# StefanDenn3r/Unsupervised_Anomaly_Detection_Brain_MRI

Hardware: AMD Instinct MI355X
Metric: MRI slices/sec VAE train step (128x128, bs=64) (higher is better)
Workload: dtype bf16x3; 1 GPU; BASELINE.json configs[1]: VAE 128x128x1 slices, batch 64 per GPU, fwd + bwd + TF-Adam (lr 1e-4, beta1 0.5), dropout 0.2, inter_res 8, zDim 128; global_batch=64, per_gpu_batch=64, parallelism=single

## Files before the change

unsupervised_anomaly_detection_brain_mri_amd/csrc/uad_misc.hip:

```cpp
#include "uad_kernels.h"
#include <stdint.h>

namespace {

__device__ __forceinline__ float wave_sum(float v) {
#pragma unroll
    for (int o = 32; o > 0; o >>= 1) v += __shfl_xor(v, o);
    return v;
}

typedef float v4f_nt __attribute__((ext_vector_type(4)));
template <int JL, int SL>
__device__ __forceinline__ void reduce4_block(v4f_nt (*red)[JL], int vb, const float* __restrict__ partial, int S, int L, float scale, float* __restrict__ out) {
    const int jl = threadIdx.x % JL, sl = threadIdx.x / JL;
    const int j4 = vb * JL + jl, L4 = L >> 2;
    v4f_nt a0 = {0.f, 0.f, 0.f, 0.f}, a1 = a0, a2 = a0, a3 = a0;
    if (j4 < L4) {
        const v4f_nt* p = reinterpret_cast<const v4f_nt*>(partial) + j4;
        int s = sl;
        for (; s + 3 * SL < S; s += 4 * SL) {
            const v4f_nt v0 = __builtin_nontemporal_load(p + (size_t)s * L4), v1 = __builtin_nontemporal_load(p + (size_t)(s + SL) * L4);
            const v4f_nt v2 = __builtin_nontemporal_load(p + (size_t)(s + 2 * SL) * L4), v3 = __builtin_nontemporal_load(p + (size_t)(s + 3 * SL) * L4);
            a0 += v0; a1 += v1; a2 += v2; a3 += v3;
        }
// ... 261 lines not shown
    else if constexpr (SLAB == RF_VEC16) reduce4_block<16, 32>(reinterpret_cast<v4f_nt (*)[16]>(lds), vb, a.partial, a.S, a.L, 1.0f, a.dW);
    else if constexpr (SLAB == RF_SCALAR4) reduce1_block<128, 4>(reinterpret_cast<float (*)[128]>(lds), vb, a.partial, a.S, a.L, 1.0f, a.dW, 1);
    else if constexpr (SLAB == RF_SCALAR16) reduce1_block<32, 16>(reinterpret_cast<float (*)[32]>(lds), vb, a.partial, a.S, a.L, 1.0f, a.dW, 1);
}

__global__ void __launch_bounds__(256) colsum_kernel(const float* __restrict__ g, int rows, int C, int rows_per_chunk,
                                                     float* __restrict__ out) {
    __shared__ float red[8][33];
    const int cl = threadIdx.x & 31, rl = threadIdx.x >> 5;
    const int c = blockIdx.x * 32 + cl;
    const int r0 = blockIdx.y * rows_per_chunk;
    const int r1 = min(r0 + rows_per_chunk, rows);
    float s = 0.f;
    if (c < C)
        for (int r = r0 + rl; r < r1; r += 8) s += g[(size_t)r * C + c];
    red[rl][cl] = s;
    __syncthreads();
    if (rl == 0 && c < C) {
        float a = 0.f;
        for (int k = 0; k < 8; ++k) a += red[k][cl];
        out[(size_t)blockIdx.y * C + c] = a;
    }
}

__global__ void __launch_bounds__(256) conv_first_fwd_kernel(UadConvDesc d, const float* __restrict__ x,
                                                             const float* __restrict__ W,
                                                             const float* __restrict__ bias, float* __restrict__ out) {
    extern __shared__ __attribute__((aligned(16))) float sm[];
    const int CS = d.CS, CB = d.CB, KS = d.KS, S = d.S, P = d.P;
    const int tpp = CS / 8;
    const int ppb = 256 / tpp;
    const int nwtaps = KS * KS * CB;
    float* ws = sm;
    const int xw = S * ppb + KS;
    float* xs = sm + nwtaps * CS;
    const int blocks_per_row = (d.WS + ppb - 1) / ppb;
    const int bx = blockIdx.x % blocks_per_row;
    const int row = blockIdx.x / blocks_per_row;
    const int n = row / d.HS, oy = row % d.HS;
    const int ox0 = bx * ppb;
    for (int i = threadIdx.x; i < nwtaps * CS; i += 256) ws[i] = W[i];
    const int ix0 = S * ox0 - P, iy0 = S * oy - P;
    for (int i = threadIdx.x; i < KS * xw * CB; i += 256) {
        const int cb = i % CB;
        const int t = i / CB;
        const int xx = t % xw, ky = t / xw;
        const int iy = iy0 + ky, ix = ix0 + xx;
        float v = 0.f;
        if ((unsigned)iy < (unsigned)d.HB && (unsigned)ix < (unsigned)d.WB)
            v = x[((size_t)(n * d.HB + iy) * d.WB + ix) * CB + cb];
        xs[i] = v;
    }
    __syncthreads();
    const int p = threadIdx.x / tpp, q = threadIdx.x % tpp;
    const int ox = ox0 + p;
    if (ox >= d.WS) return;
    float acc[8];
#pragma unroll
    for (int e = 0; e < 8; ++e) acc[e] = bias ? bias[q * 8 + e] : 0.f;
    for (int ky = 0; ky < KS; ++ky)
        for (int kx = 0; kx < KS; ++kx)
            for (int cb = 0; cb < CB; ++cb) {
                const float xv = xs[(ky * xw + S * p + kx) * CB + cb];
                const float4 w0 = *reinterpret_cast<const float4*>(ws + ((ky * KS + kx) * CB + cb) * CS + q * 8);
                const float4 w1 = *reinterpret_cast<const float4*>(ws + ((ky * KS + kx) * CB + cb) * CS + q * 8 + 4);
                acc[0] = fmaf(xv, w0.x, acc[0]); acc[1] = fmaf(xv, w0.y, acc[1]);
                acc[2] = fmaf(xv, w0.z, acc[2]); acc[3] = fmaf(xv, w0.w, acc[3]);
                acc[4] = fmaf(xv, w1.x, acc[4]); acc[5] = fmaf(xv, w1.y, acc[5]);
                acc[6] = fmaf(xv, w1.z, acc[6]); acc[7] = fmaf(xv, w1.w, acc[7]);
            }
    float* o = out + ((size_t)(n * d.HS + oy) * d.WS + ox) * CS + q * 8;
    *reinterpret_cast<float4*>(o) = make_float4(acc[0], acc[1], acc[2], acc[3]);
    *reinterpret_cast<float4*>(o + 4) = make_float4(acc[4], acc[5], acc[6], acc[7]);
}

template <int KS, int CB>
__global__ void __launch_bounds__(256) conv_first_wgrad_kernel(UadConvDesc d, const float* __restrict__ x,
                                                               const float* __restrict__ g, int rows_per_block,
                                                               float* __restrict__ partial) {
    extern __shared__ __attribute__((aligned(16))) float sm[];
    constexpr int NTAP = KS * KS * CB;
    const int CS = d.CS, S = d.S, P = d.P;
    const int G = 256 / CS;
    const int co = threadIdx.x % CS, grp = threadIdx.x / CS;
    const int xw = d.WB + KS + S;
    float* xs = sm;
    float acc[NTAP];
#pragma unroll
    for (int t = 0; t < NTAP; ++t) acc[t] = 0.f;
    const int total_rows = d.N * d.HS;
    const int row0 = blockIdx.x * rows_per_block;
    const int row1 = min(row0 + rows_per_block, total_rows);
    constexpr int RB = 4, OXB = 8;
    for (int rb = row0; rb < row1; rb += RB) {
        __syncthreads();
        for (int i = threadIdx.x; i < RB * KS * xw * CB; i += 256) {
            const int cb = i % CB;
            int t = i / CB;
            const int xx = t % xw; t /= xw;
            const int ky = t % KS, r = t / KS;
            const int row = rb + r;
            float v = 0.f;
            if (row < row1) {
                const int n = row / d.HS, oy = row % d.HS;
                const int iy = S * oy - P + ky, ix = xx - P;
                if ((unsigned)iy < (unsigned)d.HB && (unsigned)ix < (unsigned)d.WB)
                    v = x[((size_t)(n * d.HB + iy) * d.WB + ix) * CB + cb];
            }
            xs[i] = v;
        }
        __syncthreads();
        for (int ob = 0; ob < d.WS; ob += OXB * G) {
            float gv[RB][OXB];
#pragma unroll
            for (int r = 0; r < RB; ++r)
#pragma unroll
                for (int i = 0; i < OXB; ++i) {
                    const int ox = ob + grp + i * G;
                    const bool ok = (rb + r < row1) && ox < d.WS;
                    gv[r][i] = ok ? g[((size_t)(rb + r) * d.WS + ox) * CS + co] : 0.f;
                }
#pragma unroll
            for (int r = 0; r < RB; ++r)
#pragma unroll
                for (int i = 0; i < OXB; ++i) {
                    const int ox = min(ob + grp + i * G, d.WS - 1);
                    const float* xr = xs + (size_t)r * KS * xw * CB;
#pragma unroll
                    for (int ky = 0; ky < KS; ++ky)
#pragma unroll
                        for (int kx = 0; kx < KS; ++kx)
#pragma unroll
                            for (int cb = 0; cb < CB; ++cb)
                                acc[(ky * KS + kx) * CB + cb] =
                                    fmaf(xr[(ky * xw + S * ox + kx) * CB + cb], gv[r][i], acc[(ky * KS + kx) * CB + cb]);
                }
        }
    }
    __syncthreads();
    float* red = sm;
#pragma unroll
    for (int t = 0; t < NTAP; ++t) red[(grp * NTAP + t) * CS + co] = acc[t];
    __syncthreads();
    for (int i = threadIdx.x; i < NTAP * CS; i += 256) {
        float a = 0.f;
        for (int k = 0; k < G; ++k) a += red[k * NTAP * CS + i];
        partial[(size_t)blockIdx.x * NTAP * CS + i] = a;
    }
}

typedef float v2f __attribute__((ext_vector_type(2)));

template <int WS>
__global__ void __launch_bounds__(256) conv_first_fwd32_kernel(UadConvDesc d, const float* __restrict__ x, const float* __restrict__ W,
                                                               const float* __restrict__ bias, float* __restrict__ out) {
    constexpr int OR = 256 / WS, IR = 2 * OR + 3, XW = 2 * WS + 4;
    __shared__ __attribute__((aligned(16))) float ws[25 * 32];
    __shared__ __attribute__((aligned(16))) float xs[IR * XW];
    const int tid = threadIdx.x;
    const int q = tid & 3, pg = (tid >> 2) % (WS / 4), rl = tid / WS;
    const int bpi = d.HS / OR;
    const int n = blockIdx.x / bpi, oy0 = (blockIdx.x % bpi) * OR;
    for (int i = tid; i < 25 * 32; i += 256) ws[i] = W[i];
    for (int i = tid; i < IR * XW; i += 256) {
        const int r = i / XW, xx = i % XW;
        const int iy = 2 * oy0 - 1 + r, ix = xx - 1;
        xs[i] = ((unsigned)iy < (unsigned)d.HB && (unsigned)ix < (unsigned)d.WB) ? x[((size_t)n * d.HB + iy) * d.WB + ix] : 0.f;
    }
    __syncthreads();
    v2f acc[4][4];
#pragma unroll
    for (int e = 0; e < 4; ++e) {
        const v2f b = bias ? v2f{bias[q * 8 + 2 * e], bias[q * 8 + 2 * e + 1]} : v2f{0.f, 0.f};
#pragma unroll
        for (int j = 0; j < 4; ++j) acc[j][e] = b;
    }
    const float* xr0 = xs + (2 * rl) * XW + 8 * pg;
#pragma unroll
    for (int ky = 0; ky < 5; ++ky) {
        float xv[12];
#pragma unroll
        for (int k = 0; k < 3; ++k) *reinterpret_cast<float4*>(xv + 4 * k) = *reinterpret_cast<const float4*>(xr0 + ky * XW + 4 * k);
#pragma unroll
        for (int kx = 0; kx < 5; ++kx) {
            const float4 w0 = *reinterpret_cast<const float4*>(ws + (ky * 5 + kx) * 32 + q * 8);
            const float4 w1 = *reinterpret_cast<const float4*>(ws + (ky * 5 + kx) * 32 + q * 8 + 4);
            const v2f w[4] = {{w0.x, w0.y}, {w0.z, w0.w}, {w1.x, w1.y}, {w1.z, w1.w}};
#pragma unroll
            for (int j = 0; j < 4; ++j) {
                const v2f xx = {xv[2 * j + kx], xv[2 * j + kx]};
#pragma unroll
                for (int e = 0; e < 4; ++e) acc[j][e] = __builtin_elementwise_fma(xx, w[e], acc[j][e]);
            }
        }
    }
    const size_t oe = (((size_t)n * d.HS + oy0 + rl) * WS + 4 * pg) * 32 + q * 8;
    float* o = out + oe;
#pragma unroll
    for (int j = 0; j < 4; ++j) {
        *reinterpret_cast<float4*>(o + j * 32) = make_float4(acc[j][0].x, acc[j][0].y, acc[j][1].x, acc[j][1].y);
        *reinterpret_cast<float4*>(o + j * 32 + 4) = make_float4(acc[j][2].x, acc[j][2].y, acc[j][3].x, acc[j][3].y);
    }
}

template <int WS>
__global__ void __launch_bounds__(256) conv_first_wgrad32_kernel(UadConvDesc d, const float* __restrict__ x, const float* __restrict__ g,
                                                                 int RPB, float* __restrict__ partial) {
    constexpr int XW = 2 * WS + 4, NP = WS / 32, MAXR = 16;
    __shared__ __attribute__((aligned(16))) float xs[(2 * MAXR + 3) * XW];
    __shared__ __attribute__((aligned(16))) float red[4][25 * 32];
    const int tid = threadIdx.x, cq = tid & 7, pl = tid >> 3;
    const int row0 = blockIdx.x * RPB;
    const int n = row0 / d.HS, oy0 = row0 % d.HS;
    for (int i = tid; i < (2 * RPB + 3) * XW; i += 256) {
        const int r = i / XW, xx = i % XW;
        const int iy = 2 * oy0 - 1 + r, ix = xx - 1;
        xs[i] = ((unsigned)iy < (unsigned)d.HB && (unsigned)ix < (unsigned)d.WB) ? x[((size_t)n * d.HB + iy) * d.WB + ix] : 0.f;
    }
    v2f acc[25][2];
#pragma unroll
    for (int t = 0; t < 25; ++t) { acc[t][0] = v2f{0.f, 0.f}; acc[t][1] = v2f{0.f, 0.f}; }
    const float* gb = g + ((size_t)row0 * WS + pl) * 32 + cq * 4;
    float4 cur[2][NP], nxt[2][NP];
#pragma unroll
    for (int r = 0; r < 2; ++r)
#pragma unroll
        for (int k = 0; k < NP; ++k) cur[r][k] = *reinterpret_cast<const float4*>(gb + ((size_t)r * WS + k * 32) * 32);
    __syncthreads();
    for (int rp = 0; rp < RPB; rp += 2) {
        if (rp + 2 < RPB) {
#pragma unroll
            for (int r = 0; r < 2; ++r)
#pragma unroll
                for (int k = 0; k < NP; ++k) nxt[r][k] = *reinterpret_cast<const float4*>(gb + ((size_t)(rp + 2 + r) * WS + k * 32) * 32);
        }
#pragma unroll
        for (int r = 0; r < 2; ++r)
#pragma unroll
            for (int k = 0; k < NP; ++k) {
                const float* xr = xs + 2 * (rp + r) * XW + 2 * (k * 32 + pl);
                const v2f g0 = {cur[r][k].x, cur[r][k].y}, g1 = {cur[r][k].z, cur[r][k].w};
#pragma unroll
                for (int ky = 0; ky < 5; ++ky)
#pragma unroll
                    for (int kx = 0; kx < 5; ++kx) {
                        const float xv = xr[ky * XW + kx];
                        const v2f xx = {xv, xv};
                        acc[ky * 5 + kx][0] = __builtin_elementwise_fma(xx, g0, acc[ky * 5 + kx][0]);
                        acc[ky * 5 + kx][1] = __builtin_elementwise_fma(xx, g1, acc[ky * 5 + kx][1]);
                    }
            }
#pragma unroll
        for (int r = 0; r < 2; ++r)
#pragma unroll
            for (int k = 0; k < NP; ++k) cur[r][k] = nxt[r][k];
    }
#pragma unroll
    for (int t = 0; t < 25; ++t)
#pragma unroll
        for (int h = 0; h < 2; ++h) {
            float a = acc[t][h].x, b = acc[t][h].y;
            a += __shfl_xor(a, 8); b += __shfl_xor(b, 8);
            a += __shfl_xor(a, 16); b += __shfl_xor(b, 16);
            a += __shfl_xor(a, 32); b += __shfl_xor(b, 32);
            acc[t][h] = v2f{a, b};
        }
    const int wave = tid >> 6;
    if ((tid & 63) < 8) {
#pragma unroll
        for (int t = 0; t < 25; ++t)
            *reinterpret_cast<float4*>(&red[wave][t * 32 + cq * 4]) = make_float4(acc[t][0].x, acc[t][0].y, acc[t][1].x, acc[t][1].y);
    }
    __syncthreads();
    for (int i = tid; i < 25 * 32; i += 256) partial[(size_t)blockIdx.x * 800 + i] = (red[0][i] + red[1][i]) + (red[2][i] + red[3][i]);
}

template <bool BWD>
__global__ void __launch_bounds__(256) final_kernel(const UadFinalArgs a, int pix_per_block) {
    __shared__ float red[4][200];
    const int lpp = a.C / 4;
    const int ppp = 256 / lpp;
    const int cl = threadIdx.x % lpp, slot = threadIdx.x / lpp;
    const int n = blockIdx.y;
    const int hw = a.H * a.W;
    const int p0 = blockIdx.x * pix_per_block;
    const int p1 = min(p0 + pix_per_block, hw);
    float4 sc = *reinterpret_cast<const float4*>(a.scale + cl * 4);
    sc.x *= a.mult; sc.y *= a.mult; sc.z *= a.mult; sc.w *= a.mult;
    const float4 sh = *reinterpret_cast<const float4*>(a.shift + cl * 4);
    const float4 wf = *reinterpret_cast<const float4*>(a.wf + cl * 4);
    const float bf = a.bf[0];
    float rec = 0.f, dbf = 0.f;
    float dw[4] = {0, 0, 0, 0}, s1[4] = {0, 0, 0, 0}, s2[4] = {0, 0, 0, 0};
    constexpr int UNR = 4;
    auto one_pixel = [&](const size_t pix, const float4 c, const float xv) {
        float bn[4] = {fmaf(c.x, sc.x, sh.x), fmaf(c.y, sc.y, sh.y), fmaf(c.z, sc.z, sh.z), fmaf(c.w, sc.w, sh.w)};
        float av[4];
#pragma unroll
        for (int e = 0; e < 4; ++e) av[e] = bn[e] > 0.f ? bn[e] : bn[e] * a.alpha;
        float dot = av[0] * wf.x;
        dot = fmaf(av[1], wf.y, dot);
        dot = fmaf(av[2], wf.z, dot);
        dot = fmaf(av[3], wf.w, dot);
        for (int o = 1; o < lpp; o <<= 1) dot += __shfl_xor(dot, o);
        const float xh = dot + bf;
        const float diff = xh - xv;
        if (cl == 0) {
            a.x_hat[pix] = xh;
            if (a.l1_map) a.l1_map[pix] = fabsf(diff);
            rec += fabsf(diff);
        }
        if (BWD) {
            const float s = a.dxhat_in ? a.dxhat_in[pix] : (diff > 0.f ? 1.f : (diff < 0.f ? -1.f : 0.f)) * a.inv_batch;
            const float wv[4] = {wf.x, wf.y, wf.z, wf.w};
            const float cv[4] = {c.x, c.y, c.z, c.w};
            const float scv[4] = {sc.x, sc.y, sc.z, sc.w};
            float dc[4];
#pragma unroll
            for (int e = 0; e < 4; ++e) {
                const float da = s * wv[e];
                const float dbn = bn[e] > 0.f ? da : da * a.alpha;
                dc[e] = dbn * scv[e];
                dw[e] = fmaf(s, av[e], dw[e]);
                s1[e] += dbn;
                s2[e] = fmaf(dbn, cv[e], s2[e]);
            }
            *reinterpret_cast<float4*>(a.d_c + pix * a.C + cl * 4) = make_float4(dc[0], dc[1], dc[2], dc[3]);
            if (cl == 0) dbf += s;
        }
    };
    for (int p = p0 + slot; p < p1; p += ppp * UNR) {
        float4 cv[UNR];
        float xv[UNR];
#pragma unroll
        for (int u = 0; u < UNR; ++u) {
            const int pp = min(p + u * ppp, p1 - 1);
            const size_t pix = (size_t)n * hw + pp;
            cv[u] = *reinterpret_cast<const float4*>(a.c_last + pix * a.C + cl * 4);
            xv[u] = a.x[pix];
        }
#pragma unroll
        for (int u = 0; u < UNR; ++u)
            if (p + u * ppp < p1) one_pixel((size_t)n * hw + p + u * ppp, cv[u], xv[u]);
    }
    const int lane = threadIdx.x & 63, wave = threadIdx.x >> 6;
    for (int o = lpp; o < 64; o <<= 1) {
        rec += __shfl_xor(rec, o);
        if (BWD) {
            dbf += __shfl_xor(dbf, o);
#pragma unroll
            for (int e = 0; e < 4; ++e) {
                dw[e] += __shfl_xor(dw[e], o);
                s1[e] += __shfl_xor(s1[e], o);
                s2[e] += __shfl_xor(s2[e], o);
            }
        }
    }
    if (lane < lpp) {
        if (BWD) {
#pragma unroll
            for (int e = 0; e < 4; ++e) {
                red[wave][0 * a.C + lane * 4 + e] = dw[e];
                red[wave][1 * a.C + lane * 4 + e] = s1[e];
                red[wave][2 * a.C + lane * 4 + e] = s2[e];
            }
        }
        if (lane == 0) {
            red[wave][3 * a.C] = dbf;
            red[wave][3 * a.C + 1] = rec;
        }
    }
    __syncthreads();
    const int blk = blockIdx.y * gridDim.x + blockIdx.x;
    const int nred = 3 * a.C + 2;
    if ((int)threadIdx.x < nred) {
        const float v = red[0][threadIdx.x] + red[1][threadIdx.x] + red[2][threadIdx.x] + red[3][threadIdx.x];
        if ((int)threadIdx.x == 3 * a.C + 1) a.rec_partial[blk] = v;
        else if (BWD) a.red_partial[(size_t)blk * (3 * a.C + 1) + threadIdx.x] = v;
    }
}

__global__ void __launch_bounds__(64) reparam_fwd_kernel(int zdim, int n_vae, const float* __restrict__ mu_raw,
                                                         const float* __restrict__ ls_raw,
                                                         const float* __restrict__ mask_mu,
                                                         const float* __restrict__ mask_ls,
                                                         const float* __restrict__ mask_mu_ce,
                                                         const float* __restrict__ eps, float* __restrict__ mu,
                                                         float* __restrict__ ls, float* __restrict__ sigma,
                                                         float* __restrict__ z, float* __restrict__ kl) {
    const int n = blockIdx.x;
    const bool ctx = n >= n_vae;
    float acc = 0.f;
    for (int k = threadIdx.x; k < zdim; k += 64) {
        const size_t i = (size_t)n * zdim + k;
        float m = mu_raw[i];
        if (ctx) {
            if (mask_mu_ce) m *= mask_mu_ce[(size_t)(n - n_vae) * zdim + k];
            mu[i] = m; ls[i] = 0.f; sigma[i] = 1.f; z[i] = m;
            continue;
        }
        float l = ls_raw[i];
        if (mask_mu) m *= mask_mu[i];
        if (mask_ls) l *= mask_ls[i];
        const float s = expf(l);
        const float e = eps ? eps[i] : 0.f;
        mu[i] = m; ls[i] = l; sigma[i] = s;
        z[i] = fmaf(e, s, m);
        acc += m * m + s * s - 2.f * l - 1.f;
    }
    acc = wave_sum(acc);
    if (threadIdx.x == 0) kl[n] = 0.5f * acc;
}

__global__ void reparam_bwd_kernel(size_t total, int zdim, int n_vae, const float* __restrict__ dz,
                                   const float* __restrict__ mu, const float* __restrict__ sigma,
                                   const float* __restrict__ eps, const float* __restrict__ mask_mu,
                                   const float* __restrict__ mask_ls, const float* __restrict__ mask_mu_ce,
                                   float inv_batch, float* __restrict__ dmu_raw, float* __restrict__ dls_raw) {
    const size_t i = (size_t)blockIdx.x * blockDim.x + threadIdx.x;
    if (i >= total) return;
    const size_t n = i / zdim;
    const float g = dz[i];
    if (n >= (size_t)n_vae) {
        dmu_raw[i] = mask_mu_ce ? g * mask_mu_ce[i - (size_t)n_vae * zdim] : g;
        dls_raw[i] = 0.f;
// ... 303 lines not shown
namespace {
struct RngJobs { UadRngJob j[8]; };
__global__ void __launch_bounds__(256) rng_fill_kernel(RngJobs jobs, int n, unsigned k0, unsigned k1, unsigned step_lo, unsigned step_hi,
                                                       long long sample0) {
    const UadRngJob jb = jobs.j[blockIdx.y];
    const int quads = (jb.per_sample + 3) / 4;
    const long long total = (long long)n * quads;
    for (long long q = (long long)blockIdx.x * blockDim.x + threadIdx.x; q < total; q += (long long)gridDim.x * blockDim.x) {
        const int s = (int)(q / quads), e4 = (int)(q % quads);
        const unsigned long long gs = (unsigned long long)(sample0 + s);
        unsigned r[4];
        uad_rng_quad((unsigned)e4, gs, step_lo, step_hi, jb.stream, k0, k1, r);
        float v[4];
        if (jb.kind == 0) {
#pragma unroll
            for (int h = 0; h < 2; ++h) uad_box_muller(r[2 * h], r[2 * h + 1], v[2 * h], v[2 * h + 1]);
        } else {
            const float keep = 1.0f / (1.0f - jb.rate);
#pragma unroll
            for (int h = 0; h < 4; ++h) v[h] = ((float)(r[h] >> 8) * 5.9604644775390625e-8f >= jb.rate) ? keep : 0.0f;
        }
        float* o = jb.out + (size_t)s * jb.per_sample + (size_t)e4 * 4;
#pragma unroll
        for (int h = 0; h < 4; ++h) if (e4 * 4 + h < jb.per_sample) o[h] = v[h];
    }
}
}

void uad_launch_rng_fill(const UadRngJob* jobs, int njobs, int n, unsigned long long seed, unsigned long long step, long long sample0,
                         hipStream_t st) {
    RngJobs js;
    int maxq = 1;
    for (int i = 0; i < njobs; ++i) { js.j[i] = jobs[i]; const int q = (jobs[i].per_sample + 3) / 4; if (q > maxq) maxq = q; }
    long long blocks = ((long long)n * maxq + 255) / 256;
    if (blocks > 2048) blocks = 2048;
    hipLaunchKernelGGL(rng_fill_kernel, dim3((unsigned)blocks, njobs), dim3(256), 0, st, js, n, (unsigned)seed, (unsigned)(seed >> 32),
                       (unsigned)step, (unsigned)(step >> 32), sample0);
}

namespace {
__global__ void __launch_bounds__(64) clock_probe_kernel(unsigned long long* out, unsigned long long ticks) {
    const unsigned long long r0 = wall_clock64();
    const unsigned long long c0 = (unsigned long long)clock64();
    unsigned long long r = r0;
    while (r - r0 < ticks) { __builtin_amdgcn_s_sleep(64); r = wall_clock64(); }
    const unsigned long long c1 = (unsigned long long)clock64();
    if (threadIdx.x == 0) { out[0] = c1 - c0; out[1] = r - r0; }
}
}
void uad_launch_clock_probe(unsigned long long* out, unsigned long long ticks, hipStream_t st) {
    hipLaunchKernelGGL(clock_probe_kernel, dim3(1), dim3(64), 0, st, out, ticks);
}

void uad_launch_gather_slices(const float* src, const int* idx, int n, long long slice_elems, float* out, hipStream_t st) {
    const long long f4 = slice_elems / 4;
    int bx = (int)((f4 + 255) / 256); if (bx > 64) bx = 64; if (bx < 1) bx = 1;
    hipLaunchKernelGGL(gather_slices_kernel, dim3(bx, n), dim3(256), 0, st, src, idx, f4, out);
}
void uad_launch_gather_mask(const unsigned char* labels, const int* idx, int n, long long slice_px, const unsigned char* lut,
                            float* out, hipStream_t st) {
    int bx = (int)((slice_px + 255) / 256); if (bx > 64) bx = 64; if (bx < 1) bx = 1;
    hipLaunchKernelGGL(gather_mask_kernel, dim3(bx, n), dim3(256), 0, st, labels, idx, slice_px, lut, out);
}
static int reduce_form(const float* partial, int S, int L, const float* out) {
    static const bool r4 = getenv("UAD_NO_REDUCE4") == nullptr;
    if (r4 && S > 8 && L % 4 == 0 && L >= 1024 && ((uintptr_t)partial & 15) == 0 && ((uintptr_t)out & 15) == 0) {
        const int L4 = L / 4;
        return (L4 + 63) / 64 >= 256 ? RF_VEC64 : (L4 + 31) / 32 >= 256 ? RF_VEC32 : RF_VEC16;
    }
    return ((L + 63) / 64 >= 256 || S <= 8) ? RF_SCALAR4 : RF_SCALAR16;
}
void uad_launch_reduce_partials(const float* partial, int S, int L, float scale, float* out, hipStream_t st) {
    const int blocks = (L + 63) / 64, L4 = L / 4;
    constexpr int nt = 1;
    switch (reduce_form(partial, S, L, out)) {
    case RF_VEC64: hipLaunchKernelGGL((reduce_partials4_kernel<64, 8>), dim3((L4 + 63) / 64), dim3(512), 0, st, partial, S, L, scale, out); break;
    case RF_VEC32: hipLaunchKernelGGL((reduce_partials4_kernel<32, 16>), dim3((L4 + 31) / 32), dim3(512), 0, st, partial, S, L, scale, out); break;
    case RF_VEC16: hipLaunchKernelGGL((reduce_partials4_kernel<16, 32>), dim3((L4 + 15) / 16), dim3(512), 0, st, partial, S, L, scale, out); break;
    case RF_SCALAR4: hipLaunchKernelGGL((reduce_partials_kernel<4>), dim3(blocks), dim3(256), 0, st, partial, S, L, scale, out, nt); break;
    default: hipLaunchKernelGGL((reduce_partials_kernel<16>), dim3(blocks), dim3(1024), 0, st, partial, S, L, scale, out, nt); break;
    }
}

bool uad_grad_finish_takes(int C, int fin_C) { return C <= 512 && 3 * fin_C + 1 <= kFinishFinCols; }
size_t uad_grad_finish_scratch_floats() { return (size_t)kFinishBnFloats + 16 * kFinishFinCols; }
void uad_launch_grad_finish(const UadGradFinish& in, hipStream_t st) {
    UadGradFinish a = in;
    if (!a.fin_partial) a.fin_C = 0;
    if (!a.colpart) a.C = 0;
    if (!uad_grad_finish_takes(a.C, a.fin_C)) { fprintf(stderr, "uad: grad_finish does not take C = %d, fin_C = %d (uad_grad_finish_takes)\n", a.C, a.fin_C); abort(); }
    a.nfin = a.fin_partial ? (a.fin_T <= 8 ? 4 : 16) : 0;
    a.NB = a.T >= 2048 ? 32 : a.T >= 512 ? 16 : a.T >= 128 ? 8 : 1;
    a.nbn = a.colpart ? ((a.C + 31) / 32) * a.NB : 0;
    const int form = (a.partial && a.S > 0) ? reduce_form(a.partial, a.S, a.L, a.dW) : RF_NONE;
    const int L4 = a.L / 4;
    const int nslab = form == RF_VEC64 ? (L4 + 63) / 64 : form == RF_VEC32 ? (L4 + 31) / 32 : form == RF_VEC16 ? (L4 + 15) / 16
                      : form == RF_SCALAR4 ? (a.L + 127) / 128 : form == RF_SCALAR16 ? (a.L + 31) / 32 : 0;
    const dim3 grid(a.nfin + a.nbn + nslab);
    if (!grid.x) return;
    switch (form) {
    case RF_VEC64: hipLaunchKernelGGL(grad_finish_kernel<RF_VEC64>, grid, dim3(512), 0, st, a); break;
    case RF_VEC32: hipLaunchKernelGGL(grad_finish_kernel<RF_VEC32>, grid, dim3(512), 0, st, a); break;
    case RF_VEC16: hipLaunchKernelGGL(grad_finish_kernel<RF_VEC16>, grid, dim3(512), 0, st, a); break;
    case RF_SCALAR4: hipLaunchKernelGGL(grad_finish_kernel<RF_SCALAR4>, grid, dim3(512), 0, st, a); break;
    case RF_SCALAR16: hipLaunchKernelGGL(grad_finish_kernel<RF_SCALAR16>, grid, dim3(512), 0, st, a); break;
    default: hipLaunchKernelGGL(grad_finish_kernel<RF_NONE>, grid, dim3(512), 0, st, a); break;
    }
}

void uad_launch_final_gradfin(const float* red, int C, const float* gamma, float rstd, float* dwf, float* dbf, float* dgamma, float* dbeta,
                              float* dbias, hipStream_t st) {
    hipLaunchKernelGGL(final_gradfin_kernel, dim3(1), dim3(256), 0, st, red, C, gamma, rstd, dwf, dbf, dgamma, dbeta, dbias);
}
size_t uad_bn_grad_finalize_scratch_floats(int C) { return 64 + (size_t)((C + 31) / 32) * 32 * 64; }
void uad_launch_bn_grad_finalize(const float* colpart, int T, int C, const float* gamma, float rstd, float* dgamma,
                                 float* dbeta, float* dbias, hipStream_t st, float* scratch) {
    const int NB = T >= 2048 ? 32 : T >= 512 ? 16 : T >= 128 ? 8 : 1;
    if (scratch && NB > 1 && C <= 512) {
        hipLaunchKernelGGL(bn_grad_finalize2_kernel, dim3((C + 31) / 32, NB), dim3(1024), 0, st, colpart, T, C, gamma, rstd, dgamma, dbeta, dbias, scratch);
        return;
    }
    hipLaunchKernelGGL(bn_grad_finalize_kernel, dim3((C + 31) / 32), dim3(1024), 0, st, colpart, T, C, gamma, rstd,
                       dgamma, dbeta, dbias);
}

static inline int colsum_chunks(int rows, int C) {
    static const int cap_env = getenv("UAD_COLSUM_CHUNKS") ? atoi(getenv("UAD_COLSUM_CHUNKS")) : 0;
    int cap = cap_env > 0 ? cap_env : 1024;
    const int fit = (int)kUadColsumScratchFloats / (C < 1 ? 1 : C);
    if (cap > fit) cap = fit;
    if (cap < 1) cap = 1;
    int ch = (rows + 255) / 256;
    return ch < 1 ? 1 : (ch > cap ? cap : ch);
}
size_t uad_colsum_scratch_floats(int rows, int C) { return (size_t)colsum_chunks(rows, C) * C; }

void uad_launch_colsum(const float* g, int rows, int C, float* out, float* scratch, hipStream_t st) {
    const int ch = colsum_chunks(rows, C);
    const int rpc = (rows + ch - 1) / ch;
    dim3 grid((C + 31) / 32, ch);
    if (ch == 1) {
        hipLaunchKernelGGL(colsum_kernel, grid, dim3(256), 0, st, g, rows, C, rpc, out);
    } else {
        hipLaunchKernelGGL(colsum_kernel, grid, dim3(256), 0, st, g, rows, C, rpc, scratch);
        uad_launch_reduce_partials(scratch, ch, C, 1.0f, out, st);
    }
}

static inline bool first32_ok(const UadConvDesc& d) {
    static const bool off = getenv("UAD_NO_FIRST32") != nullptr;
    return !off && d.CB == 1 && d.CS == 32 && d.KS == 5 && d.S == 2 && d.P == 1 && d.HB == 2 * d.HS && d.WB == 2 * d.WS &&
           (d.WS == 32 || d.WS == 64 || d.WS == 128) && d.HS % 8 == 0;
}
void uad_launch_conv_first_fwd(const UadConvDesc& d, const float* x, const float* W, const float* bias, float* out,
                               hipStream_t st) {
    const int tpp = d.CS / 8, ppb = 256 / tpp;
    const int xw = d.S * ppb + d.KS;
    const size_t lds = ((size_t)d.KS * d.KS * d.CB * d.CS + (size_t)d.KS * xw * d.CB) * sizeof(float);
    const int bpr = (d.WS + ppb - 1) / ppb;
    if (first32_ok(d)) {
        if (d.WS == 32) hipLaunchKernelGGL(conv_first_fwd32_kernel<32>, dim3(d.N * d.HS / 8), dim3(256), 0, st, d, x, W, bias, out);
        else if (d.WS == 64) hipLaunchKernelGGL(conv_first_fwd32_kernel<64>, dim3(d.N * d.HS / 4), dim3(256), 0, st, d, x, W, bias, out);
        else hipLaunchKernelGGL(conv_first_fwd32_kernel<128>, dim3(d.N * d.HS / 2), dim3(256), 0, st, d, x, W, bias, out);
        return;
    }
    hipLaunchKernelGGL(conv_first_fwd_kernel, dim3(d.N * d.HS * bpr), dim3(256), lds, st, d, x, W, bias, out);
}

static inline int first_wgrad_rows_per_block(const UadConvDesc& d) {
    const int total = d.N * d.HS;
    if (first32_ok(d)) {
        const int want = (total + 511) / 512;
        return (want > 8 && d.HS % 16 == 0) ? 16 : want > 4 ? 8 : 4;
    }
    int rpb = (total + 1023) / 1024;
    return rpb < 1 ? 1 : rpb;
}
size_t uad_conv_first_wgrad_partial_floats(const UadConvDesc& d) {
    const int rpb = first_wgrad_rows_per_block(d);
    const int blocks = (d.N * d.HS + rpb - 1) / rpb;
    return (size_t)blocks * d.KS * d.KS * d.CB * d.CS;
}
void uad_launch_conv_first_wgrad(const UadConvDesc& d, const float* x, const float* g, float* dW, float* partial,
                                 hipStream_t st) {
    const int rpb = first_wgrad_rows_per_block(d);
    const int blocks = (d.N * d.HS + rpb - 1) / rpb;
    const int ntap = d.KS * d.KS * d.CB;
    const int G = 256 / d.CS;
    const int xw = d.WB + d.KS + d.S;
    size_t lds_x = (size_t)4 * d.KS * xw * d.CB, lds_r = (size_t)G * ntap * d.CS;
    const size_t lds = (lds_x > lds_r ? lds_x : lds_r) * sizeof(float);
    if (first32_ok(d)) {
        if (d.WS == 32) hipLaunchKernelGGL(conv_first_wgrad32_kernel<32>, dim3(blocks), dim3(256), 0, st, d, x, g, rpb, partial);
        else if (d.WS == 64) hipLaunchKernelGGL(conv_first_wgrad32_kernel<64>, dim3(blocks), dim3(256), 0, st, d, x, g, rpb, partial);
        else hipLaunchKernelGGL(conv_first_wgrad32_kernel<128>, dim3(blocks), dim3(256), 0, st, d, x, g, rpb, partial);
    } else if (d.KS == 5 && d.CB == 1)
        hipLaunchKernelGGL((conv_first_wgrad_kernel<5, 1>), dim3(blocks), dim3(256), lds, st, d, x, g, rpb, partial);
    else if (d.KS == 5 && d.CB == 3)
        hipLaunchKernelGGL((conv_first_wgrad_kernel<5, 3>), dim3(blocks), dim3(256), lds, st, d, x, g, rpb, partial);
    else if (d.KS == 3 && d.CB == 1)
        hipLaunchKernelGGL((conv_first_wgrad_kernel<3, 1>), dim3(blocks), dim3(256), lds, st, d, x, g, rpb, partial);
    else if (d.KS == 4 && d.CB == 1)
        hipLaunchKernelGGL((conv_first_wgrad_kernel<4, 1>), dim3(blocks), dim3(256), lds, st, d, x, g, rpb, partial);
    else
        return;
    uad_launch_reduce_partials(partial, blocks, ntap * d.CS, 1.0f, dW, st);
}

int uad_final_blocks_per_sample(int H, int W) {
    const int hw = H * W;
    int bps = hw / 512;
    return bps < 1 ? 1 : bps;
}
void uad_launch_final_fwd_bwd(const UadFinalArgs& a, hipStream_t st) {
    const int bps = uad_final_blocks_per_sample(a.H, a.W);
    const int ppb = (a.H * a.W + bps - 1) / bps;
    dim3 grid(bps, a.N);
    if (a.d_c)
        hipLaunchKernelGGL((final_kernel<true>), grid, dim3(256), 0, st, a, ppb);
    else
        hipLaunchKernelGGL((final_kernel<false>), grid, dim3(256), 0, st, a, ppb);
}

void uad_launch_reparam_fwd(int n, int n_vae, int zdim, const float* mu_raw, const float* ls_raw, const float* mask_mu,
                            const float* mask_ls, const float* mask_mu_ce, const float* eps, float* mu, float* ls,
                            float* sigma, float* z, float* kl_per_sample, hipStream_t st) {
    hipLaunchKernelGGL(reparam_fwd_kernel, dim3(n), dim3(64), 0, st, zdim, n_vae, mu_raw, ls_raw, mask_mu, mask_ls,
                       mask_mu_ce, eps, mu, ls, sigma, z, kl_per_sample);
}
void uad_launch_reparam_bwd(int n, int n_vae, int zdim, const float* dz, const float* mu, const float* sigma,
                            const float* eps, const float* mask_mu, const float* mask_ls, const float* mask_mu_ce,
                            float inv_batch, float* dmu_raw, float* dls_raw, hipStream_t st) {
    const size_t total = (size_t)n * zdim;
    hipLaunchKernelGGL(reparam_bwd_kernel, dim3((total + 255) / 256), dim3(256), 0, st, total, zdim, n_vae, dz, mu,
                       sigma, eps, mask_mu, mask_ls, mask_mu_ce, inv_batch, dmu_raw, dls_raw);
}
static bool first_dgrad_tiled_ok(const UadConvDesc& d) {
    return d.KS == 5 && d.S == 2 && d.P == 1 && d.CB == 1 && d.CS == 32 && d.HB % 16 == 0 && d.WB % 16 == 0 &&
           d.HB == 2 * d.HS && d.WB == 2 * d.WS && d.N <= 65535;
}
void uad_launch_conv_first_dgrad(const UadConvDesc& d, const float* g, const float* W, const float* x,
                                 const float* x_hat, float inv_batch, float* anomaly, float* dx, hipStream_t st) {
    if (first_dgrad_tiled_ok(d)) {
        FirstDgradEpi e{x, x_hat, inv_batch, anomaly, dx, nullptr, nullptr, 0.f};
        hipLaunchKernelGGL(conv_first_dgrad_tiled_kernel, dim3(d.WB / 16, d.HB / 16, d.N), dim3(256), 0, st, d, g, W, e);
        return;
    }
    const size_t total = (size_t)d.N * d.HB * d.WB;
    hipLaunchKernelGGL(conv_first_dgrad_kernel, dim3((total + 255) / 256), dim3(256),
                       (size_t)d.KS * d.KS * d.CS * sizeof(float), st, d, g, W, x, x_hat, inv_batch, anomaly, dx,
                       (const float*)nullptr, (float*)nullptr, 0.f);
}
void uad_launch_conv_first_dgrad_restore(const UadConvDesc& d, const float* g, const float* W, const float* dxhat,
                                         float* dx, float* x_upd, float restore_lr, hipStream_t st) {
    if (first_dgrad_tiled_ok(d)) {
        FirstDgradEpi e{nullptr, nullptr, 0.f, nullptr, dx, dxhat, x_upd, restore_lr};
        hipLaunchKernelGGL(conv_first_dgrad_tiled_kernel, dim3(d.WB / 16, d.HB / 16, d.N), dim3(256), 0, st, d, g, W, e);
        return;
    }
    const size_t total = (size_t)d.N * d.HB * d.WB;
    hipLaunchKernelGGL(conv_first_dgrad_kernel, dim3((total + 255) / 256), dim3(256),
                       (size_t)d.KS * d.KS * d.CS * sizeof(float), st, d, g, W, (const float*)nullptr,
                       (const float*)nullptr, 0.f, (float*)nullptr, dx, dxhat, x_upd, restore_lr);
}
void uad_launch_conv_first_dgrad_plain(const UadConvDesc& d, const float* g, const float* W, float* dx, hipStream_t st) {
    uad_launch_conv_first_dgrad(d, g, W, nullptr, nullptr, 0.f, nullptr, dx, st);
}
void uad_launch_mul(const float* x, const float* mask, float* y, size_t n, hipStream_t st) {
    hipLaunchKernelGGL(mul_kernel, dim3((n + 255) / 256), dim3(256), 0, st, x, mask, y, n);
}
void uad_launch_loss_finalize(const float* rec_partial, int n, int n_vae, int bps, const float* kl_per_sample,
                              float inv_batch, float rec_scale, float* rec_per_sample, float* scalars, hipStream_t st) {
    hipLaunchKernelGGL(loss_finalize_kernel, dim3(1), dim3(256), 0, st, rec_partial, n, n_vae, bps, kl_per_sample,
                       inv_batch, rec_scale, rec_per_sample, scalars);
}
void uad_launch_optim(int kind, float* p, const float* g, float* s1, float* s2, size_t n, float lr, float momentum, float decay, float eps,
                      float gscale, hipStream_t st, const unsigned* fault) {
    hipLaunchKernelGGL(optim_kernel, dim3((n + 255) / 256), dim3(256), 0, st, kind, p, g, s1, s2, n, lr, momentum, decay, eps, gscale, fault);
}
void uad_launch_adam(float* p, const float* g, float* m, float* v, size_t n, float lr_t, float beta1, float beta2,
                     float eps, float gscale, hipStream_t st, const unsigned* fault) {
    hipLaunchKernelGGL(adam_kernel, dim3((n + 255) / 256), dim3(256), 0, st, p, g, m, v, n, lr_t, beta1, beta2, eps,
                       gscale, fault);
}
void uad_launch_residual(const float* x, const float* xr, const float* mask, int n, int hw, int pos_only,
                         float prior_thresh, float* out, float* l1err, hipStream_t st) {
    hipLaunchKernelGGL(residual_kernel, dim3(1, n), dim3(256), 0, st, x, xr, mask, hw, pos_only, prior_thresh, out,
                       l1err);
}
```

Measured before the change: 79930 slices/s.

## Restructure first-layer conv fwd/wgrad kernels with vectorized staging and register weights

Rewrites the 5x5 stride-2 first-conv forward kernel so each thread keeps its 4 output channels' weights in registers and loops over pixels, and stages input rows with float4 loads into padded LDS. The weight-gradient kernel gets a compile-time rows-per-block, a deeper register ring for prefetching gradients, and a transpose-style shuffle reduction that halves the data exchanged at each step. The rows-per-block threshold also shifts so larger blocks are used at the boundary. Adds an alignment check that falls back to the generic kernels, plus more register pressure and template instantiations.

Measured after the change: 80560 slices/s (median of 6 runs). Within noise of the previous version (+0.8%).

```diff
diff --git a/unsupervised_anomaly_detection_brain_mri_amd/csrc/uad_misc.hip b/unsupervised_anomaly_detection_brain_mri_amd/csrc/uad_misc.hip
--- a/unsupervised_anomaly_detection_brain_mri_amd/csrc/uad_misc.hip
+++ b/unsupervised_anomaly_detection_brain_mri_amd/csrc/uad_misc.hip
@@ -437,125 +437,129 @@
 typedef float v2f __attribute__((ext_vector_type(2)));
 
 template <int WS>
+__device__ __forceinline__ void first32_stage_rows(float* __restrict__ xs, const float* __restrict__ xn, int iy0, int nrows, int HB, int tid) {
+    constexpr int XS = 2 * WS + 8, C4 = WS / 2;
+    for (int i = tid; i < nrows * C4; i += 256) {
+        const int r = i / C4, c = i % C4;
+        const int iy = iy0 + r;
+        float4 v = make_float4(0.f, 0.f, 0.f, 0.f);
+        if ((unsigned)iy < (unsigned)HB) v = *reinterpret_cast<const float4*>(xn + (size_t)iy * (2 * WS) + 4 * c);
+        *reinterpret_cast<float4*>(xs + r * XS + 4 + 4 * c) = v;
+    }
+    if (tid < nrows) {
+        xs[tid * XS + 3] = 0.f;
+        xs[tid * XS + 2 * WS + 4] = 0.f;
+        xs[tid * XS + 2 * WS + 5] = 0.f;
+    }
+}
+
+template <int WS>
 __global__ void __launch_bounds__(256) conv_first_fwd32_kernel(UadConvDesc d, const float* __restrict__ x, const float* __restrict__ W,
                                                                const float* __restrict__ bias, float* __restrict__ out) {
-    constexpr int OR = 256 / WS, IR = 2 * OR + 3, XW = 2 * WS + 4;
+    constexpr int OR = 256 / WS, IR = 2 * OR + 3, XS = 2 * WS + 8;
     __shared__ __attribute__((aligned(16))) float ws[25 * 32];
-    __shared__ __attribute__((aligned(16))) float xs[IR * XW];
+    __shared__ __attribute__((aligned(16))) float xs[IR * XS];
     const int tid = threadIdx.x;
-    const int q = tid & 3, pg = (tid >> 2) % (WS / 4), rl = tid / WS;
+    const int cq = tid & 7, pl = tid >> 3;
     const int bpi = d.HS / OR;
     const int n = blockIdx.x / bpi, oy0 = (blockIdx.x % bpi) * OR;
     for (int i = tid; i < 25 * 32; i += 256) ws[i] = W[i];
-    for (int i = tid; i < IR * XW; i += 256) {
-        const int r = i / XW, xx = i % XW;
-        const int iy = 2 * oy0 - 1 + r, ix = xx - 1;
-        xs[i] = ((unsigned)iy < (unsigned)d.HB && (unsigned)ix < (unsigned)d.WB) ? x[((size_t)n * d.HB + iy) * d.WB + ix] : 0.f;
-    }
-    __syncthreads();
-    v2f acc[4][4];
-#pragma unroll
-    for (int e = 0; e < 4; ++e) {
-        const v2f b = bias ? v2f{bias[q * 8 + 2 * e], bias[q * 8 + 2 * e + 1]} : v2f{0.f, 0.f};
-#pragma unroll
-        for (int j = 0; j < 4; ++j) acc[j][e] = b;
-    }
-    const float* xr0 = xs + (2 * rl) * XW + 8 * pg;
-#pragma unroll
-    for (int ky = 0; ky < 5; ++ky) {
-        float xv[12];
-#pragma unroll
-        for (int k = 0; k < 3; ++k) *reinterpret_cast<float4*>(xv + 4 * k) = *reinterpret_cast<const float4*>(xr0 + ky * XW + 4 * k);
-#pragma unroll
-        for (int kx = 0; kx < 5; ++kx) {
-            const float4 w0 = *reinterpret_cast<const float4*>(ws + (ky * 5 + kx) * 32 + q * 8);
-            const float4 w1 = *reinterpret_cast<const float4*>(ws + (ky * 5 + kx) * 32 + q * 8 + 4);
-            const v2f w[4] = {{w0.x, w0.y}, {w0.z, w0.w}, {w1.x, w1.y}, {w1.z, w1.w}};
-#pragma unroll
-            for (int j = 0; j < 4; ++j) {
-                const v2f xx = {xv[2 * j + kx], xv[2 * j + kx]};
-#pragma unroll
-                for (int e = 0; e < 4; ++e) acc[j][e] = __builtin_elementwise_fma(xx, w[e], acc[j][e]);
+    first32_stage_rows<WS>(xs, x + (size_t)n * d.HB * (2 * WS), 2 * oy0 - 1, IR, d.HB, tid);
+    const v2f b0 = bias ? v2f{bias[cq * 4], bias[cq * 4 + 1]} : v2f{0.f, 0.f};
+    const v2f b1 = bias ? v2f{bias[cq * 4 + 2], bias[cq * 4 + 3]} : v2f{0.f, 0.f};
+    __syncthreads();
+    v2f w0[25], w1[25];
+#pragma unroll
+    for (int t = 0; t < 25; ++t) {
+        const float4 w = *reinterpret_cast<const float4*>(ws + t * 32 + cq * 4);
+        w0[t] = v2f{w.x, w.y}; w1[t] = v2f{w.z, w.w};
+    }
+    float* ob = out + ((size_t)n * d.HS + oy0) * WS * 32 + cq * 4;
+#pragma unroll 2
+    for (int j = 0; j < 8; ++j) {
+        const int p = j * 32 + pl;
+        const float* xr = xs + 2 * (p / WS) * XS + 2 * (p % WS) + 3;
+        v2f a0 = b0, a1 = b1;
+#pragma unroll
+        for (int ky = 0; ky < 5; ++ky) {
+            const float xa = xr[ky * XS];
+            const float2 xb = *reinterpret_cast<const float2*>(xr + ky * XS + 1);
+            const float2 xc = *reinterpret_cast<const float2*>(xr + ky * XS + 3);
+            const float xv[5] = {xa, xb.x, xb.y, xc.x, xc.y};
+#pragma unroll
+            for (int kx = 0; kx < 5; ++kx) {
+                const v2f xx = {xv[kx], xv[kx]};
+                a0 = __builtin_elementwise_fma(xx, w0[ky * 5 + kx], a0);
+                a1 = __builtin_elementwise_fma(xx, w1[ky * 5 + kx], a1);
             }
         }
-    }
-    const size_t oe = (((size_t)n * d.HS + oy0 + rl) * WS + 4 * pg) * 32 + q * 8;
-    float* o = out + oe;
-#pragma unroll
-    for (int j = 0; j < 4; ++j) {
-        *reinterpret_cast<float4*>(o + j * 32) = make_float4(acc[j][0].x, acc[j][0].y, acc[j][1].x, acc[j][1].y);
-        *reinterpret_cast<float4*>(o + j * 32 + 4) = make_float4(acc[j][2].x, acc[j][2].y, acc[j][3].x, acc[j][3].y);
-    }
-}
-
-template <int WS>
+        *reinterpret_cast<float4*>(ob + (size_t)p * 32) = make_float4(a0.x, a0.y, a1.x, a1.y);
+    }
+}
+
+template <int WS, int RPB>
 __global__ void __launch_bounds__(256) conv_first_wgrad32_kernel(UadConvDesc d, const float* __restrict__ x, const float* __restrict__ g,
-                                                                 int RPB, float* __restrict__ partial) {
-    constexpr int XW = 2 * WS + 4, NP = WS / 32, MAXR = 16;
-    __shared__ __attribute__((aligned(16))) float xs[(2 * MAXR + 3) * XW];
+                                                                 float* __restrict__ partial) {
+    constexpr int XS = 2 * WS + 8, NP = WS / 32, IR = 2 * RPB + 3, NL = RPB * NP, DEPTH = NL <= 16 ? NL : 8;
+    static_assert(DEPTH % NP == 0 && NL % DEPTH == 0, "the ring holds whole rows and divides the block");
+    __shared__ __attribute__((aligned(16))) float xs[IR * XS];
     __shared__ __attribute__((aligned(16))) float red[4][25 * 32];
     const int tid = threadIdx.x, cq = tid & 7, pl = tid >> 3;
     const int row0 = blockIdx.x * RPB;
     const int n = row0 / d.HS, oy0 = row0 % d.HS;
-    for (int i = tid; i < (2 * RPB + 3) * XW; i += 256) {
-        const int r = i / XW, xx = i % XW;
-        const int iy = 2 * oy0 - 1 + r, ix = xx - 1;
-        xs[i] = ((unsigned)iy < (unsigned)d.HB && (unsigned)ix < (unsigned)d.WB) ? x[((size_t)n * d.HB + iy) * d.WB + ix] : 0.f;
-    }
+    const float* gb = g + ((size_t)row0 * WS + pl) * 32 + cq * 4;
+    float4 ring[DEPTH];
+#pragma unroll
+    for (int s = 0; s < DEPTH; ++s) ring[s] = *reinterpret_cast<const float4*>(gb + ((size_t)(s / NP) * WS + (s % NP) * 32) * 32);
+    first32_stage_rows<WS>(xs, x + (size_t)n * d.HB * (2 * WS), 2 * oy0 - 1, IR, d.HB, tid);
     v2f acc[25][2];
 #pragma unroll
     for (int t = 0; t < 25; ++t) { acc[t][0] = v2f{0.f, 0.f}; acc[t][1] = v2f{0.f, 0.f}; }
-    const float* gb = g + ((size_t)row0 * WS + pl) * 32 + cq * 4;
-    float4 cur[2][NP], nxt[2][NP];
-#pragma unroll
-    for (int r = 0; r < 2; ++r)
-#pragma unroll
-        for (int k = 0; k < NP; ++k) cur[r][k] = *reinterpret_cast<const float4*>(gb + ((size_t)r * WS + k * 32) * 32);
-    __syncthreads();
-    for (int rp = 0; rp < RPB; rp += 2) {
-        if (rp + 2 < RPB) {
-#pragma unroll
-            for (int r = 0; r < 2; ++r)
-#pragma unroll
-                for (int k = 0; k < NP; ++k) nxt[r][k] = *reinterpret_cast<const float4*>(gb + ((size_t)(rp + 2 + r) * WS + k * 32) * 32);
-        }
-#pragma unroll
-        for (int r = 0; r < 2; ++r)
-#pragma unroll
-            for (int k = 0; k < NP; ++k) {
-                const float* xr = xs + 2 * (rp + r) * XW + 2 * (k * 32 + pl);
-                const v2f g0 = {cur[r][k].x, cur[r][k].y}, g1 = {cur[r][k].z, cur[r][k].w};
-#pragma unroll
-                for (int ky = 0; ky < 5; ++ky)
-#pragma unroll
-                    for (int kx = 0; kx < 5; ++kx) {
-                        const float xv = xr[ky * XW + kx];
-                        const v2f xx = {xv, xv};
-                        acc[ky * 5 + kx][0] = __builtin_elementwise_fma(xx, g0, acc[ky * 5 + kx][0]);
-                        acc[ky * 5 + kx][1] = __builtin_elementwise_fma(xx, g1, acc[ky * 5 + kx][1]);
-                    }
+    __syncthreads();
+    auto accumulate = [&](const float4 gv, const float* xr) {
+        const v2f g0 = {gv.x, gv.y}, g1 = {gv.z, gv.w};
+#pragma unroll
+        for (int ky = 0; ky < 5; ++ky) {
+            const float xa = xr[ky * XS];
+            const float2 xb = *reinterpret_cast<const float2*>(xr + ky * XS + 1);
+            const float2 xc = *reinterpret_cast<const float2*>(xr + ky * XS + 3);
+            const float xv[5] = {xa, xb.x, xb.y, xc.x, xc.y};
+#pragma unroll
+            for (int kx = 0; kx < 5; ++kx) {
+                const v2f xx = {xv[kx], xv[kx]};
+                acc[ky * 5 + kx][0] = __builtin_elementwise_fma(xx, g0, acc[ky * 5 + kx][0]);
+                acc[ky * 5 + kx][1] = __builtin_elementwise_fma(xx, g1, acc[ky * 5 + kx][1]);
             }
-#pragma unroll
-        for (int r = 0; r < 2; ++r)
-#pragma unroll
-            for (int k = 0; k < NP; ++k) cur[r][k] = nxt[r][k];
-    }
-#pragma unroll
-    for (int t = 0; t < 25; ++t)
-#pragma unroll
-        for (int h = 0; h < 2; ++h) {
-            float a = acc[t][h].x, b = acc[t][h].y;
-            a += __shfl_xor(a, 8); b += __shfl_xor(b, 8);
-            a += __shfl_xor(a, 16); b += __shfl_xor(b, 16);
-            a += __shfl_xor(a, 32); b += __shfl_xor(b, 32);
-            acc[t][h] = v2f{a, b};
-        }
+        }
+    };
+    const float* xp = xs + 2 * pl + 3;
+#pragma unroll 1
+    for (int r0 = 0; r0 < RPB - DEPTH / NP; r0 += DEPTH / NP) {
+#pragma unroll
+        for (int s = 0; s < DEPTH; ++s) {
+            const float4 gv = ring[s];
+            ring[s] = *reinterpret_cast<const float4*>(gb + ((size_t)(r0 + (s + DEPTH) / NP) * WS + (s % NP) * 32) * 32);
+            accumulate(gv, xp + 2 * (r0 + s / NP) * XS + (s % NP) * 64);
+        }
+    }
+#pragma unroll
+    for (int s = 0; s < DEPTH; ++s) accumulate(ring[s], xp + 2 * (RPB - DEPTH / NP + s / NP) * XS + (s % NP) * 64);
+    float v[100];
+#pragma unroll
+    for (int t = 0; t < 25; ++t) { v[4 * t] = acc[t][0].x; v[4 * t + 1] = acc[t][0].y; v[4 * t + 2] = acc[t][1].x; v[4 * t + 3] = acc[t][1].y; }
+    const bool hA = tid & 32, hB = tid & 16, hC = tid & 8;
+#pragma unroll
+    for (int i = 0; i < 50; ++i) { const float send = hA ? v[i] : v[i + 50], keep = hA ? v[i + 50] : v[i]; v[i] = keep + __shfl_xor(send, 32); }
+#pragma unroll
+    for (int i = 0; i < 25; ++i) { const float send = hB ? v[i] : v[i + 25], keep = hB ? v[i + 25] : v[i]; v[i] = keep + __shfl_xor(send, 16); }
+#pragma unroll
+    for (int i = 0; i < 12; ++i) { const float send = hC ? v[i] : v[i + 13], keep = hC ? v[i + 13] : v[i]; v[i] = keep + __shfl_xor(send, 8); }
+    v[12] += __shfl_xor(v[12], 8);
     const int wave = tid >> 6;
-    if ((tid & 63) < 8) {
-#pragma unroll
-        for (int t = 0; t < 25; ++t)
-            *reinterpret_cast<float4*>(&red[wave][t * 32 + cq * 4]) = make_float4(acc[t][0].x, acc[t][0].y, acc[t][1].x, acc[t][1].y);
-    }
+    const int e0 = (hA ? 50 : 0) + (hB ? 25 : 0);
+#pragma unroll
+    for (int i = 0; i < 12; ++i) { const int e = e0 + (hC ? 13 : 0) + i; red[wave][(e >> 2) * 32 + cq * 4 + (e & 3)] = v[i]; }
+    if (!hC) { const int e = e0 + 12; red[wave][(e >> 2) * 32 + cq * 4 + (e & 3)] = v[12]; }
     __syncthreads();
     for (int i = tid; i < 25 * 32; i += 256) partial[(size_t)blockIdx.x * 800 + i] = (red[0][i] + red[1][i]) + (red[2][i] + red[3][i]);
 }
@@ -1165,13 +1169,14 @@
     return !off && d.CB == 1 && d.CS == 32 && d.KS == 5 && d.S == 2 && d.P == 1 && d.HB == 2 * d.HS && d.WB == 2 * d.WS &&
            (d.WS == 32 || d.WS == 64 || d.WS == 128) && d.HS % 8 == 0;
 }
+static inline bool first32_aligned(const float* x) { return ((uintptr_t)x & 15) == 0; }
 void uad_launch_conv_first_fwd(const UadConvDesc& d, const float* x, const float* W, const float* bias, float* out,
                                hipStream_t st) {
     const int tpp = d.CS / 8, ppb = 256 / tpp;
     const int xw = d.S * ppb + d.KS;
     const size_t lds = ((size_t)d.KS * d.KS * d.CB * d.CS + (size_t)d.KS * xw * d.CB) * sizeof(float);
     const int bpr = (d.WS + ppb - 1) / ppb;
-    if (first32_ok(d)) {
+    if (first32_ok(d) && first32_aligned(x)) {
         if (d.WS == 32) hipLaunchKernelGGL(conv_first_fwd32_kernel<32>, dim3(d.N * d.HS / 8), dim3(256), 0, st, d, x, W, bias, out);
         else if (d.WS == 64) hipLaunchKernelGGL(conv_first_fwd32_kernel<64>, dim3(d.N * d.HS / 4), dim3(256), 0, st, d, x, W, bias, out);
         else hipLaunchKernelGGL(conv_first_fwd32_kernel<128>, dim3(d.N * d.HS / 2), dim3(256), 0, st, d, x, W, bias, out);
@@ -1184,29 +1189,34 @@
     const int total = d.N * d.HS;
     if (first32_ok(d)) {
         const int want = (total + 511) / 512;
-        return (want > 8 && d.HS % 16 == 0) ? 16 : want > 4 ? 8 : 4;
+        return (want >= 8 && d.HS % 16 == 0) ? 16 : want > 4 ? 8 : 4;
     }
     int rpb = (total + 1023) / 1024;
     return rpb < 1 ? 1 : rpb;
 }
+static inline int first_wgrad_blocks(const UadConvDesc& d, int rpb) { return (d.N * d.HS + rpb - 1) / rpb; }
 size_t uad_conv_first_wgrad_partial_floats(const UadConvDesc& d) {
-    const int rpb = first_wgrad_rows_per_block(d);
-    const int blocks = (d.N * d.HS + rpb - 1) / rpb;
-    return (size_t)blocks * d.KS * d.KS * d.CB * d.CS;
+    return (size_t)first_wgrad_blocks(d, first_wgrad_rows_per_block(d)) * d.KS * d.KS * d.CB * d.CS;
+}
+template <int WS>
+static void launch_first_wgrad32(const UadConvDesc& d, const float* x, const float* g, int rpb, int blocks, float* partial, hipStream_t st) {
+    if (rpb == 4) hipLaunchKernelGGL((conv_first_wgrad32_kernel<WS, 4>), dim3(blocks), dim3(256), 0, st, d, x, g, partial);
+    else if (rpb == 8) hipLaunchKernelGGL((conv_first_wgrad32_kernel<WS, 8>), dim3(blocks), dim3(256), 0, st, d, x, g, partial);
+    else hipLaunchKernelGGL((conv_first_wgrad32_kernel<WS, 16>), dim3(blocks), dim3(256), 0, st, d, x, g, partial);
 }
 void uad_launch_conv_first_wgrad(const UadConvDesc& d, const float* x, const float* g, float* dW, float* partial,
                                  hipStream_t st) {
     const int rpb = first_wgrad_rows_per_block(d);
-    const int blocks = (d.N * d.HS + rpb - 1) / rpb;
+    const int blocks = first_wgrad_blocks(d, rpb);
     const int ntap = d.KS * d.KS * d.CB;
     const int G = 256 / d.CS;
     const int xw = d.WB + d.KS + d.S;
     size_t lds_x = (size_t)4 * d.KS * xw * d.CB, lds_r = (size_t)G * ntap * d.CS;
     const size_t lds = (lds_x > lds_r ? lds_x : lds_r) * sizeof(float);
-    if (first32_ok(d)) {
-        if (d.WS == 32) hipLaunchKernelGGL(conv_first_wgrad32_kernel<32>, dim3(blocks), dim3(256), 0, st, d, x, g, rpb, partial);
-        else if (d.WS == 64) hipLaunchKernelGGL(conv_first_wgrad32_kernel<64>, dim3(blocks), dim3(256), 0, st, d, x, g, rpb, partial);
-        else hipLaunchKernelGGL(conv_first_wgrad32_kernel<128>, dim3(blocks), dim3(256), 0, st, d, x, g, rpb, partial);
+    if (first32_ok(d) && first32_aligned(x)) {
+        if (d.WS == 32) launch_first_wgrad32<32>(d, x, g, rpb, blocks, partial, st);
+        else if (d.WS == 64) launch_first_wgrad32<64>(d, x, g, rpb, blocks, partial, st);
+        else launch_first_wgrad32<128>(d, x, g, rpb, blocks, partial, st);
     } else if (d.KS == 5 && d.CB == 1)
         hipLaunchKernelGGL((conv_first_wgrad_kernel<5, 1>), dim3(blocks), dim3(256), lds, st, d, x, g, rpb, partial);
     else if (d.KS == 5 && d.CB == 3)
```
